# ag14774/MPILattice-Boltzmann

Measured on AMD Instinct MI355X. Metric: MLUPS, higher is better.
Workload: dtype f32; 1 GPU; synthetic 8192x8192 D2Q9-BGK deck (walls + p=0.005 random obstacles, splitmix64 seed 42), density 0.1 accel 0.005 omega 1.85; nx=8192, ny=8192, partitioning=single GPU, loop=single, macro_k=0, launches_per_exchange=1, step_allreduce=False, kernel=lbm_multi_kernel<4>

## Files before the change

### mpilattice-boltzmann_amd/csrc/kernels/multi.h

```cpp
#pragma once
#include "common.h"

namespace {

#ifndef LBM_MTY
#define LBM_MTY 16
#define LBM_MLANES 512
#endif
#ifndef LBM_MWAVES
#define LBM_MWAVES 6
#endif
#ifndef LBM_MTY4
#define LBM_MTY4 13
#endif
#ifndef LBM_MTY4T
#define LBM_MTY4T 24
#define LBM_MLANES4T 768
#endif
constexpr int kMTX = 64, kMTXNarrow = 32, kMTY = LBM_MTY, kMTY4 = LBM_MTY4, kMTY4Tall = LBM_MTY4T, kMLanes = LBM_MLANES, kMLanes4Tall = LBM_MLANES4T,
              kMaxMultiSteps = 4,
              kMaxGhost = 32,
              kMaxGroup = 8;
constexpr int kMinMultiTY = kMTY < kMTY4 ? (kMTY < kMTY4Tall ? kMTY : kMTY4Tall) : (kMTY4 < kMTY4Tall ? kMTY4 : kMTY4Tall);
constexpr int kGeomStd = 0, kGeomNarrow = 1, kGeomTall = 2;
constexpr int geom_tx(int g) { return g == kGeomNarrow ? kMTXNarrow : kMTX; }
constexpr int multi_ty(int k, int g) { return k >= 4 ? (g == kGeomTall ? kMTY4Tall : kMTY4) : kMTY; }
constexpr int multi_lanes(int k, int g) { return (k >= 4 && g == kGeomTall) ? kMLanes4Tall : kMLanes; }
constexpr int geom_for(int k, int g) { return (g == kGeomTall && k < 4) ? kGeomStd : g; }

constexpr int multi_ex(int ey) { return 2 * ((ey + 1) / 2); }
#if LBM_TILE_STAMPS
#define LBM_MSTAMP(i) do { if (blockIdx.x == (gridDim.x >> 1) && threadIdx.x == 0) g_tile_stamps[i] = __builtin_amdgcn_s_memtime(); } while (0)
#else
#define LBM_MSTAMP(i) do { } while (0)
#endif

template <int K, int GEOM = kGeomStd>
struct MultiGeom {
  static constexpr int TX = geom_tx(GEOM);
  static constexpr int TY = multi_ty(K, GEOM);
  static constexpr int LANES = multi_lanes(K, GEOM);
  static constexpr int EY = K - 1, EX = multi_ex(K - 1);
  static constexpr int W = TX + 2 * EX, H = TY + 2 * EY;
  static constexpr int cells = W * H;
  static constexpr size_t lds_bytes = sizeof(float) * 9 * cells + sizeof(double) * K * (LANES / 64) + (K >= 2 ? cells / 2 : 0);
  static constexpr int blocks_per_cu = lds_bytes * 8 <= 160 * 1024 ? 8 : static_cast<int>(160 * 1024 / lds_bytes);
  static constexpr int waves_per_simd = blocks_per_cu * (LANES / 64) / 4 < LBM_MWAVES ? (blocks_per_cu * (LANES / 64) / 4 < 1 ? 1 : blocks_per_cu * (LANES / 64) / 4) : LBM_MWAVES;
};

struct MultiArgs {
  const float* src;
  float* dst;
  const float* srck[9];
  float* dstk[9];
  const uint32_t* mask;
  size_t ps;
  int nx;
  int row_first, rows_compute;
  int rows_storage;
  int count_first, count_end;
  int y_periodic;
  int y0_global, ny_global;
  int tiles_x;
  int tile_begin, tile_count, tile_begin2, tile_count2;
  int ntiles_total;
  int xcd_remap;
  float omega, accel_w1, accel_w2;
  int accel_row;
  int accel_last;
  double* partials_out;
  const double* prev_partials;
  int n_prev, n_prev_vecs;
  double* sums;
  int* counter;
  unsigned long long* ready[2];
  unsigned long long ready_epoch;
  const unsigned long long* wait_ready;
  long long timeout_ticks;
  int* err;
  int keep_x0, keep_x1, cx0, cx1;
  unsigned long long* ready_x[2];
  int nrect;
  struct Rect { int ty0, tx0, ntx, count; } rect[4];
  int nblocks;
};

template <int W>
__device__ __forceinline__ void store_pair(float* plane, int k, int row, int fx, f2 v)
{
  if (k == 0 || k == 2 || k == 4) {
    *reinterpret_cast<f2*>(plane + row + fx) = v;
  } else {
    plane[row + (fx >> 1)] = v.y;
    plane[row + (fx >> 1) + W / 2] = v.x;
  }
}

constexpr int kPartPlain = 0, kPartGhost = 1, kPartReady = 2, kPartTile = 3;
template <int K, int TERMS, int GEOM, int PART>
__global__ void __launch_bounds__((MultiGeom<K, GEOM>::LANES), (MultiGeom<K, GEOM>::waves_per_simd)) lbm_multi_kernel(const MultiArgs a)
{
  using G = MultiGeom<K, GEOM>;
  constexpr int TX = G::TX, EX = G::EX, EY = G::EY, W = G::W, WH = G::W / 2, kCells = G::cells, kLanes = G::LANES, kWaves = kLanes / 64, TY = G::TY;
  extern __shared__ __attribute__((aligned(16))) float lds[];
  double* red = reinterpret_cast<double*>(lds + 9 * kCells);
  uint8_t* pair_flags = reinterpret_cast<uint8_t*>(red + K * kWaves);
  const int tid = threadIdx.x;

  if (blockIdx.x == 0) {
    if constexpr (PART == kPartReady) {
      if (a.ready_epoch != 0ull && tid == 0) {
        for (int d = 0; d < 2; ++d) __hip_atomic_store(a.ready[d], a.ready_epoch, __ATOMIC_RELAXED, __HIP_MEMORY_SCOPE_SYSTEM);
      }
    }
    if constexpr (PART == kPartTile) {
      if (a.ready_epoch != 0ull && tid == 0) {
        for (int d = 0; d < 2; ++d) __hip_atomic_store(a.ready[d], a.ready_epoch, __ATOMIC_RELAXED, __HIP_MEMORY_SCOPE_SYSTEM);
        for (int d = 0; d < 2; ++d) __hip_atomic_store(a.ready_x[d], a.ready_epoch, __ATOMIC_RELAXED, __HIP_MEMORY_SCOPE_SYSTEM);
      }
    }
    for (int v = 0; v < a.n_prev_vecs; ++v) {
      double s = 0.0;
      for (int i = tid; i < a.n_prev; i += kLanes) s += a.prev_partials[static_cast<size_t>(v) * a.n_prev + i];
      s = wave_sum(s);
      __syncthreads();
      if ((tid & 63) == 0) red[tid >> 6] = s;
      __syncthreads();
      if (tid == 0) {
        double t = 0.0;
        for (int w = 0; w < kWaves; ++w) t += red[w];
        a.sums[*a.counter + v] = t;
      }
    }
    __syncthreads();
    if (tid == 0 && a.n_prev_vecs > 0) *a.counter += a.n_prev_vecs;
    if constexpr (PART == kPartReady) {
      if (a.wait_ready && tid == 0) p2p_wait_flags(a.wait_ready, nullptr, 2, a.ready_epoch, 0ull, a.timeout_ticks, a.err, false);
    }
    if constexpr (PART == kPartTile) {
      if (a.wait_ready && tid == 0) p2p_wait_flags(a.wait_ready, nullptr, 4, a.ready_epoch, 0ull, a.timeout_ticks, a.err, false);
    }
    return;
  }

  LBM_MSTAMP(0);
  int b = blockIdx.x - 1;
  if (a.xcd_remap) {
    const int nb = gridDim.x - 1, per = nb >> 3;
    b = (b & 7) * per + (b >> 3);
  }
  if constexpr (PART == kPartTile) {
    if (b >= a.nblocks) return;
  }
  int tile_of_block = b < a.tile_count ? a.tile_begin + b : a.tile_begin2 + (b - a.tile_count);
  if constexpr (PART == kPartTile) {
    if (a.nrect > 0) {
      int q = b, ty0 = a.rect[0].ty0, tx0 = a.rect[0].tx0, ntx = a.rect[0].ntx;
      if (a.nrect > 1 && q >= a.rect[0].count) {
        q -= a.rect[0].count; ty0 = a.rect[1].ty0; tx0 = a.rect[1].tx0; ntx = a.rect[1].ntx;
        if (a.nrect > 2 && q >= a.rect[1].count) {
          q -= a.rect[1].count; ty0 = a.rect[2].ty0; tx0 = a.rect[2].tx0; ntx = a.rect[2].ntx;
          if (a.nrect > 3 && q >= a.rect[2].count) { q -= a.rect[2].count; ty0 = a.rect[3].ty0; tx0 = a.rect[3].tx0; ntx = a.rect[3].ntx; }
        }
      }
      const int rr = q / ntx;
      tile_of_block = (ty0 + rr) * a.tiles_x + tx0 + (q - rr * ntx);
    }
  }
  const int tile = tile_of_block;
  const int ty = tile / a.tiles_x, tx = tile - ty * a.tiles_x;
  const int x0 = tx * TX;
  const int sy0 = a.row_first + ty * TY;
  const int nx = a.nx;
  constexpr bool XR = PART == kPartTile;
  const int rows_storage = (PART == kPartGhost || PART == kPartTile) ? a.rows_storage : a.rows_compute + 2 * a.row_first;
  [[maybe_unused]] const int row_end = a.row_first + a.rows_compute;
  const int tile_row_base = sy0 * nx;
  const int grid_cells = rows_storage * nx;
  constexpr int ksteps = K;
  double acc[K];
  float acc_lo[K];
#pragma unroll
  for (int i = 0; i < K; ++i) { acc[i] = 0.0; acc_lo[i] = 0.0f; }

  bool tile_accel;
  {
    int d = (a.accel_row - (a.y0_global + ty * TY - EY)) % a.ny_global;
    if (d < 0) d += a.ny_global;
    tile_accel = d < G::H || a.ny_global < G::H;
  }
  auto on_accel_row = [&](int sr) {
    int g = a.y0_global + sr - a.row_first;
    if (g < 0) g += a.ny_global; else if (g >= a.ny_global) g -= a.ny_global;
    return g == a.accel_row;
  };

  auto k_substeps = [&](auto count_c) __attribute__((always_inline)) {
    constexpr bool COUNT = decltype(count_c)::value;
    {
      const int ey = ksteps - 1, ex = multi_ex(ey);
      const int wp = (TX + 2 * ex) / 2;
      const int np = wp * (TY + 2 * ey);
      const bool inner = x0 - EX >= 2 && x0 + TX + EX + 2 <= nx && sy0 - EY >= 1 && sy0 + TY + EY + 1 <= rows_storage &&
                         sy0 + TY <= a.row_first + a.rows_compute;
  #pragma unroll 1
      for (int i = tid; i < np; i += kLanes) {
        const int ry = i / wp, rp = i - ry * wp;
        const int fx = EX - ex + 2 * rp, fy = EY - ey + ry;
        int gx = x0 + fx - EX;
        int sr = sy0 + fy - EY;
        int cell = tile_row_base + __mul24(fy - EY, nx) + gx;
        int d_south = -nx, d_north = nx;
        if (!inner) {
          if (gx < 0) { gx += nx; cell += nx; } else if (gx >= nx) { gx -= nx; cell -= nx; }
          if (!a.y_periodic && sr + 1 >= rows_storage) {
            if (ksteps > 1) pair_flags[(fy * W + fx) >> 1] = 0;
            continue;
          }
          if (a.y_periodic) {
            if (sr < 0) { sr += rows_storage; cell += grid_cells; } else if (sr >= rows_storage) { sr -= rows_storage; cell -= grid_cells; }
            if (sr == 0) d_south = grid_cells - nx;
            if (sr + 1 >= rows_storage) d_north = nx - grid_cells;
          }
        }
        const uint32_t o_here = 4u * static_cast<uint32_t>(cell);
        const uint32_t o_south = 4u * static_cast<uint32_t>(cell + d_south);
        const uint32_t o_north = 4u * static_cast<uint32_t>(cell + d_north);
        f2 p[9];
        p[0] = at_byte<f2>(a.srck[0], o_here);
        p[2] = at_byte<f2>(a.srck[2], o_south);
        p[4] = at_byte<f2>(a.srck[4], o_north);
        p[1] = at_byte<f2u>(a.srck[1] - 1, o_here);
        p[5] = at_byte<f2u>(a.srck[5] - 1, o_south);
        p[8] = at_byte<f2u>(a.srck[8] - 1, o_north);
        p[3] = at_byte<f2u>(a.srck[3] + 1, o_here);
        p[6] = at_byte<f2u>(a.srck[6] + 1, o_south);
        p[7] = at_byte<f2u>(a.srck[7] + 1, o_north);
        if (!inner) {
          if (gx == 0) {
            p[1].x = at_byte<float>(a.srck[1] + nx - 1, o_here); p[5].x = at_byte<float>(a.srck[5] + nx - 1, o_south);
            p[8].x = at_byte<float>(a.srck[8] + nx - 1, o_north);
          }
          if (gx == nx - 2) {
            p[3].y = at_byte<float>(a.srck[3] + 2 - nx, o_here); p[6].y = at_byte<float>(a.srck[6] + 2 - nx, o_south);
            p[7].y = at_byte<float>(a.srck[7] + 2 - nx, o_north);
          }
        }
        const uint32_t mbits = (at_byte<uint32_t>(a.mask, 4u * (static_cast<uint32_t>(cell) >> 5)) >> (cell & 31)) & 3u;
        f2 out[9];
        const int srow = sy0 + fy - EY;
        const bool owned_rows = fx >= EX && fx < EX + TX && fy >= EY && fy < EY + TY &&
                                (inner || (x0 + fx - EX < nx && sy0 + fy - EY < a.row_first + a.rows_compute));
        const bool counted_rows = COUNT ? (owned_rows && srow >= a.count_first && srow < a.count_end) : owned_rows;
        bool owned = owned_rows, counted = counted_rows;
        if constexpr (XR && COUNT) {
          const int gxo = x0 + fx - EX;
          owned = owned_rows && gxo >= a.keep_x0 && gxo < a.keep_x1;
          counted = counted_rows && owned && gxo >= a.cx0 && gxo < a.cx1;
        }
        bool accel_row_here = false;
        if (tile_accel) accel_row_here = on_accel_row(sr);
        acc[0] += finish_pair_lo<TERMS>(p, mbits, a.omega, tile_accel, (ksteps > 1 || a.accel_last) && accel_row_here, a.accel_w1, a.accel_w2, counted ? mbits : 3u, out, acc_lo[0]);
        if (ksteps > 1) {
  #pragma unroll
          for (int k = 0; k < 9; ++k) store_pair<W>(lds + k * kCells, k, fy * W, fx, out[k]);
          pair_flags[(fy * W + fx) >> 1] = static_cast<uint8_t>(mbits | (owned ? 4u : 0u) | (accel_row_here ? 8u : 0u) | 16u | ((COUNT && counted) ? 32u : 0u));
        } else if (owned) {
  #pragma unroll
          for (int k = 0; k < 9; ++k) __builtin_nontemporal_store(out[k], &at_byte<f2>(a.dstk[k], o_here));
        }
      }
    }
    LBM_MSTAMP(1);
    if constexpr (K >= 2) {
      __syncthreads();
      LBM_MSTAMP(2);
      auto in_lds_substep = [&](const int j) __attribute__((always_inline)) {
        const int ey = ksteps - j, ex = multi_ex(ey);
        const int wp = (TX + 2 * ex) / 2;
        const int rows = TY + 2 * ey;
        const int rpp = kLanes / wp;
        const bool last = j == ksteps;
        const int rd = (j - 2) * W, wr = (j - 1) * W;
        const int ry = tid / wp, rp = tid - ry * wp;
        const int fx = EX - ex + 2 * rp;
        for (int r0 = 0; r0 < rows; r0 += rpp) {
          f2 outs[9];
          int slot = -1;
          const bool in_region = ry < rpp && r0 + ry < rows;
          if (__builtin_amdgcn_ballot_w64(in_region) != 0ull) {
            const int fy = EY - ey + (in_region ? r0 + ry : 0);
            const int cf = fy * W + fx;
            const uint32_t fl = pair_flags[cf >> 1];
            const bool lane_on = in_region && (fl & 16u);
            const int ci = cf - rd;
            const int cs = fy * W + (fx >> 1) - rd;
            f2 p[9];
            p[0] = *reinterpret_cast<const f2*>(lds + 0 * kCells + ci);
            p[2] = *reinterpret_cast<const f2*>(lds + 2 * kCells + ci - W);
            p[4] = *reinterpret_cast<const f2*>(lds + 4 * kCells + ci + W);
            p[1] = f2{lds[1 * kCells + cs - 1], lds[1 * kCells + cs + WH]};
            p[5] = f2{lds[5 * kCells + cs - W - 1], lds[5 * kCells + cs - W + WH]};
            p[8] = f2{lds[8 * kCells + cs + W - 1], lds[8 * kCells + cs + W + WH]};
            p[3] = f2{lds[3 * kCells + cs], lds[3 * kCells + cs + WH + 1]};
            p[6] = f2{lds[6 * kCells + cs - W], lds[6 * kCells + cs - W + WH + 1]};
            p[7] = f2{lds[7 * kCells + cs + W], lds[7 * kCells + cs + W + WH + 1]};
            const bool owned = lane_on && (fl & 4u);
            const bool counted = COUNT ? (lane_on && (fl & 32u)) : owned;
            float term_lo = 0.0f;
            const double term = finish_pair_lo<TERMS>(p, fl & 3u, a.omega, tile_accel, (!last || a.accel_last) && (fl & 8u), a.accel_w1, a.accel_w2,
                                                      counted ? (fl & 3u) : 3u, outs, term_lo);
  #pragma unroll
            for (int m = 1; m < K; ++m)
              if (m == j - 1) { acc[m] += term; acc_lo[m] += term_lo; }
            slot = !lane_on ? -1 : last ? (owned ? tile_row_base + __mul24(fy - EY, nx) + x0 + fx - EX : -1) : fy * W - wr;
          }
          if (!last) {
            __syncthreads();
            if (slot >= 0) {
  #pragma unroll
              for (int k = 0; k < 9; ++k) store_pair<W>(lds + k * kCells, k, slot, fx, outs[k]);
            }
          } else if (slot >= 0) {
  #pragma unroll
            for (int k = 0; k < 9; ++k) __builtin_nontemporal_store(outs[k], &at_byte<f2>(a.dstk[k], 4u * static_cast<uint32_t>(slot)));
          }
        }
        if (!last) __syncthreads();
        LBM_MSTAMP(1 + j);
      };
  #pragma unroll
      for (int j = 2; j <= K; ++j) in_lds_substep(j);
    }

  };
  if constexpr (PART == kPartGhost) {
    if (sy0 >= a.count_first && sy0 + TY <= a.count_end) k_substeps(std::false_type{});
    else k_substeps(std::true_type{});
  } else if constexpr (PART == kPartTile) {
    if (sy0 >= a.count_first && sy0 + TY <= a.count_end && x0 >= a.cx0 && x0 + TX <= a.cx1) k_substeps(std::false_type{});
    else k_substeps(std::true_type{});
  } else {
    k_substeps(std::false_type{});
  }

  if constexpr (TERMS == kTermsCompensated) {
#pragma unroll
    for (int i = 0; i < K; ++i) acc[i] += static_cast<double>(acc_lo[i]);
  }
  if constexpr (K == 1) {
    const double w = wave_sum(acc[0]);
    if ((tid & 63) == 0) red[tid >> 6] = w;
  } else {
    static_assert(K <= 4, "wave_sum_vec4 carries four steps");
    const double w = wave_sum_vec4(acc[0], acc[1], K > 2 ? acc[2] : 0.0, K > 3 ? acc[K > 3 ? 3 : 0] : 0.0);
    const int q = wave_sum_slot<4>(tid & 63);
    if ((tid & 15) == 0 && q < K) red[q * kWaves + (tid >> 6)] = w;
  }
  lds_barrier();
  if (tid < ksteps) {
    double t = 0.0;
    for (int w = 0; w < kWaves; ++w) t += red[tid * kWaves + w];
    a.partials_out[static_cast<size_t>(tid) * a.ntiles_total + tile] = t;
  }
  LBM_MSTAMP(2 + K);
}

}
```

Before: 239,700 MLUPS.

## Keep owned cell pairs in registers across fused substeps for K=4 tall tiles

Adds an owned-lanes path for the K=4 tall geometry. Each lane owns one interior cell pair for all substeps and keeps its rest population in a register, while a shrinking halo ring is recomputed by the remaining lanes. Flags for owned cells stay in registers, and the loop over the halo is replaced by at most one ring pair per lane. This is meant to cut LDS traffic, loop overhead and index math, at the cost of extra register pressure and a second barrier per substep.

```diff
diff --git a/mpilattice-boltzmann_amd/csrc/kernels/multi.h b/mpilattice-boltzmann_amd/csrc/kernels/multi.h
--- a/mpilattice-boltzmann_amd/csrc/kernels/multi.h
+++ b/mpilattice-boltzmann_amd/csrc/kernels/multi.h
@@ -46,6 +46,8 @@
   static constexpr size_t lds_bytes = sizeof(float) * 9 * cells + sizeof(double) * K * (LANES / 64) + (K >= 2 ? cells / 2 : 0);
   static constexpr int blocks_per_cu = lds_bytes * 8 <= 160 * 1024 ? 8 : static_cast<int>(160 * 1024 / lds_bytes);
   static constexpr int waves_per_simd = blocks_per_cu * (LANES / 64) / 4 < LBM_MWAVES ? (blocks_per_cu * (LANES / 64) / 4 < 1 ? 1 : blocks_per_cu * (LANES / 64) / 4) : LBM_MWAVES;
+  static constexpr bool owned_lanes = K == 4 && GEOM == kGeomTall;
+  static constexpr int ring_pairs(int j) { return 2 * (K - j) * (TX / 2 + multi_ex(K - j)) + TY * multi_ex(K - j); }
 };
 
 struct MultiArgs {
@@ -96,6 +98,16 @@
   }
 }
 
+__device__ __forceinline__ void accelerate_pair(f2 (&out)[9], uint32_t mbits, bool accel, float w1, float w2)
+{
+#pragma unroll
+  for (int j = 0; j < 2; ++j) {
+    const bool go = accel && !((mbits >> j) & 1u) && out[3][j] - w1 > 0.0f && out[6][j] - w2 > 0.0f && out[7][j] - w2 > 0.0f;
+    out[1][j] = go ? out[1][j] + w1 : out[1][j]; out[5][j] = go ? out[5][j] + w2 : out[5][j]; out[8][j] = go ? out[8][j] + w2 : out[8][j];
+    out[3][j] = go ? out[3][j] - w1 : out[3][j]; out[6][j] = go ? out[6][j] - w2 : out[6][j]; out[7][j] = go ? out[7][j] - w2 : out[7][j];
+  }
+}
+
 constexpr int kPartPlain = 0, kPartGhost = 1, kPartReady = 2, kPartTile = 3;
 template <int K, int TERMS, int GEOM, int PART>
 __global__ void __launch_bounds__((MultiGeom<K, GEOM>::LANES), (MultiGeom<K, GEOM>::waves_per_simd)) lbm_multi_kernel(const MultiArgs a)
@@ -195,14 +207,15 @@
     return g == a.accel_row;
   };
 
+  const bool inner = x0 - EX >= 2 && x0 + TX + EX + 2 <= nx && sy0 - EY >= 1 && sy0 + TY + EY + 1 <= rows_storage &&
+                     sy0 + TY <= a.row_first + a.rows_compute;
+
   auto k_substeps = [&](auto count_c) __attribute__((always_inline)) {
     constexpr bool COUNT = decltype(count_c)::value;
     {
       const int ey = ksteps - 1, ex = multi_ex(ey);
       const int wp = (TX + 2 * ex) / 2;
       const int np = wp * (TY + 2 * ey);
-      const bool inner = x0 - EX >= 2 && x0 + TX + EX + 2 <= nx && sy0 - EY >= 1 && sy0 + TY + EY + 1 <= rows_storage &&
-                         sy0 + TY <= a.row_first + a.rows_compute;
   #pragma unroll 1
       for (int i = tid; i < np; i += kLanes) {
         const int ry = i / wp, rp = i - ry * wp;
@@ -334,17 +347,184 @@
     }
 
   };
+
+  auto owned_substeps = [&](auto count_c) __attribute__((always_inline)) {
+    constexpr bool COUNT = decltype(count_c)::value;
+    constexpr int TP = TX / 2;
+    static_assert(TP * TY == kLanes && G::ring_pairs(1) <= kLanes, "one owned pair and at most one ring pair per lane and sub-step");
+    auto ring_pos = [&](auto jc, const int i, int& fx, int& fy) __attribute__((always_inline)) {
+      constexpr int ey = K - decltype(jc)::value, ex = multi_ex(ey), ep = ex / 2, wp = TP + ep * 2, band = ey * wp;
+      if (i < 2 * band) {
+        const bool top = i >= band;
+        const int q = top ? i - band : i, ry = q / wp, rp = q - ry * wp;
+        fy = top ? EY + TY + ry : EY - ey + ry;
+        fx = EX - ex + 2 * rp;
+      } else {
+        const int q = i - 2 * band, ry = q / (2 * ep), c = q - ry * (2 * ep);
+        fy = EY + ry;
+        fx = EX - ex + 2 * (c < ep ? c : c + TP);
+      }
+    };
+    auto relax = [&](const f2 (&p)[9], const uint32_t mbits, const bool accel, const uint32_t skip, f2 (&out)[9]) __attribute__((always_inline)) {
+      const double term = finish_pair<TERMS>(p, mbits, a.omega, false, false, a.accel_w1, a.accel_w2, skip, out);
+      if (tile_accel) accelerate_pair(out, mbits, accel, a.accel_w1, a.accel_w2);
+      return term;
+    };
+    auto pull = [&](const int fx, const int fy, f2 (&p)[9], uint32_t& mbits, int& sr) __attribute__((always_inline)) -> bool {
+      int gx = x0 + fx - EX;
+      sr = sy0 + fy - EY;
+      int cell = tile_row_base + __mul24(fy - EY, nx) + gx;
+      int d_south = -nx, d_north = nx;
+      if (!inner) {
+        if (gx < 0) { gx += nx; cell += nx; } else if (gx >= nx) { gx -= nx; cell -= nx; }
+        if (!a.y_periodic && sr + 1 >= rows_storage) return false;
+        if (a.y_periodic) {
+          if (sr < 0) { sr += rows_storage; cell += grid_cells; } else if (sr >= rows_storage) { sr -= rows_storage; cell -= grid_cells; }
+          if (sr == 0) d_south = grid_cells - nx;
+          if (sr + 1 >= rows_storage) d_north = nx - grid_cells;
+        }
+      }
+      const uint32_t o_here = 4u * static_cast<uint32_t>(cell);
+      const uint32_t o_south = 4u * static_cast<uint32_t>(cell + d_south);
+      const uint32_t o_north = 4u * static_cast<uint32_t>(cell + d_north);
+      p[0] = at_byte<f2>(a.srck[0], o_here);
+      p[2] = at_byte<f2>(a.srck[2], o_south);
+      p[4] = at_byte<f2>(a.srck[4], o_north);
+      p[1] = at_byte<f2u>(a.srck[1] - 1, o_here);
+      p[5] = at_byte<f2u>(a.srck[5] - 1, o_south);
+      p[8] = at_byte<f2u>(a.srck[8] - 1, o_north);
+      p[3] = at_byte<f2u>(a.srck[3] + 1, o_here);
+      p[6] = at_byte<f2u>(a.srck[6] + 1, o_south);
+      p[7] = at_byte<f2u>(a.srck[7] + 1, o_north);
+      if (!inner) {
+        if (gx == 0) {
+          p[1].x = at_byte<float>(a.srck[1] + nx - 1, o_here); p[5].x = at_byte<float>(a.srck[5] + nx - 1, o_south);
+          p[8].x = at_byte<float>(a.srck[8] + nx - 1, o_north);
+        }
+        if (gx == nx - 2) {
+          p[3].y = at_byte<float>(a.srck[3] + 2 - nx, o_here); p[6].y = at_byte<float>(a.srck[6] + 2 - nx, o_south);
+          p[7].y = at_byte<float>(a.srck[7] + 2 - nx, o_north);
+        }
+      }
+      mbits = (at_byte<uint32_t>(a.mask, 4u * (static_cast<uint32_t>(cell) >> 5)) >> (cell & 31)) & 3u;
+      return true;
+    };
+    const int py = tid / TP, ofx = EX + 2 * (tid - py * TP), ofy = EY + py;
+    f2 own0 = f2{0.0f, 0.0f};
+    uint32_t ofl = 0;
+  #pragma unroll 1
+    for (int item = 0; item < 2; ++item) {
+      const bool own = item == 0;
+      if (!own && tid >= G::ring_pairs(1)) break;
+      int fx = ofx, fy = ofy;
+      if (!own) ring_pos(std::integral_constant<int, 1>{}, tid, fx, fy);
+      f2 p[9];
+      uint32_t mbits = 0, fl = 0;
+      int sr = 0;
+      if (pull(fx, fy, p, mbits, sr)) {
+        const int srow = sy0 + fy - EY;
+        const bool kept_rows = own && (inner || (x0 + fx - EX < nx && srow < a.row_first + a.rows_compute));
+        const bool counted_rows = COUNT ? (kept_rows && srow >= a.count_first && srow < a.count_end) : kept_rows;
+        bool kept = kept_rows, counted = counted_rows;
+        if constexpr (XR && COUNT) {
+          const int gxo = x0 + fx - EX;
+          kept = kept_rows && gxo >= a.keep_x0 && gxo < a.keep_x1;
+          counted = counted_rows && kept && gxo >= a.cx0 && gxo < a.cx1;
+        }
+        bool accel_row_here = false;
+        if (tile_accel) accel_row_here = on_accel_row(sr);
+        f2 out[9];
+        const double term = relax(p, mbits, accel_row_here, counted ? mbits : 3u, out);
+  #pragma unroll
+        for (int k = 1; k < 9; ++k) store_pair<W>(lds + k * kCells, k, fy * W, fx, out[k]);
+        fl = mbits | (kept ? 4u : 0u) | (accel_row_here ? 8u : 0u) | 16u | ((COUNT && counted) ? 32u : 0u);
+        if (own) {
+          acc[0] = term;
+          own0 = out[0];
+        } else {
+          store_pair<W>(lds, 0, fy * W, fx, out[0]);
+        }
+      }
+      if (own) ofl = fl;
+      else pair_flags[(fy * W + fx) >> 1] = static_cast<uint8_t>(fl);
+    }
+    LBM_MSTAMP(1);
+    __syncthreads();
+    LBM_MSTAMP(2);
+    auto in_lds_substep = [&](auto jc) __attribute__((always_inline)) {
+      constexpr int j = decltype(jc)::value;
+      constexpr bool last = j == K;
+      constexpr int rd = (j - 2) * W, wr = (j - 1) * W;
+      auto read_pair = [&](const int fx, const int fy, f2 (&p)[9]) __attribute__((always_inline)) {
+        const int ci = fy * W + fx - rd, cs = fy * W + (fx >> 1) - rd;
+        p[2] = *reinterpret_cast<const f2*>(lds + 2 * kCells + ci - W);
+        p[4] = *reinterpret_cast<const f2*>(lds + 4 * kCells + ci + W);
+        p[1] = f2{lds[1 * kCells + cs - 1], lds[1 * kCells + cs + WH]};
+        p[5] = f2{lds[5 * kCells + cs - W - 1], lds[5 * kCells + cs - W + WH]};
+        p[8] = f2{lds[8 * kCells + cs + W - 1], lds[8 * kCells + cs + W + WH]};
+        p[3] = f2{lds[3 * kCells + cs], lds[3 * kCells + cs + WH + 1]};
+        p[6] = f2{lds[6 * kCells + cs - W], lds[6 * kCells + cs - W + WH + 1]};
+        p[7] = f2{lds[7 * kCells + cs + W], lds[7 * kCells + cs + W + WH + 1]};
+      };
+      f2 p[9], outs[9];
+      read_pair(ofx, ofy, p);
+      p[0] = own0;
+      const uint32_t mbits = ofl & 3u;
+      const bool counted = COUNT ? (ofl & 32u) != 0u : (ofl & 4u) != 0u;
+      acc[j - 1] = relax(p, mbits, (!last || a.accel_last) && (ofl & 8u), counted ? mbits : 3u, outs);
+      own0 = outs[0];
+      if constexpr (!last) {
+        f2 q[9];
+        int rfx = 0, rfy = 0;
+        uint32_t rfl = 0;
+        const bool ring = tid < G::ring_pairs(j);
+        if (ring) {
+          ring_pos(jc, tid, rfx, rfy);
+          rfl = pair_flags[(rfy * W + rfx) >> 1];
+          read_pair(rfx, rfy, q);
+          q[0] = *reinterpret_cast<const f2*>(lds + rfy * W + rfx - rd);
+        }
+        __syncthreads();
+        if (ofl & 16u) {
+  #pragma unroll
+          for (int k = 1; k < 9; ++k) store_pair<W>(lds + k * kCells, k, ofy * W - wr, ofx, outs[k]);
+        }
+        if (ring) {
+          f2 routs[9];
+          relax(q, rfl & 3u, (rfl & 8u) != 0u, 3u, routs);
+          if (rfl & 16u) {
+  #pragma unroll
+            for (int k = 0; k < 9; ++k) store_pair<W>(lds + k * kCells, k, rfy * W - wr, rfx, routs[k]);
+          }
+        }
+        __syncthreads();
+      } else if (ofl & 4u) {
+        const uint32_t o = 4u * static_cast<uint32_t>(tile_row_base + __mul24(py, nx) + x0 + ofx - EX);
+  #pragma unroll
+        for (int k = 0; k < 9; ++k) __builtin_nontemporal_store(outs[k], &at_byte<f2>(a.dstk[k], o));
+      }
+      LBM_MSTAMP(1 + j);
+    };
+    in_lds_substep(std::integral_constant<int, 2>{});
+    if constexpr (K >= 3) in_lds_substep(std::integral_constant<int, K >= 3 ? 3 : 2>{});
+    if constexpr (K >= 4) in_lds_substep(std::integral_constant<int, K >= 4 ? 4 : 2>{});
+  };
+  auto substeps = [&](auto count_c) __attribute__((always_inline)) {
+    if constexpr (G::owned_lanes) owned_substeps(count_c);
+    else k_substeps(count_c);
+  };
+
   if constexpr (PART == kPartGhost) {
-    if (sy0 >= a.count_first && sy0 + TY <= a.count_end) k_substeps(std::false_type{});
-    else k_substeps(std::true_type{});
+    if (sy0 >= a.count_first && sy0 + TY <= a.count_end) substeps(std::false_type{});
+    else substeps(std::true_type{});
   } else if constexpr (PART == kPartTile) {
-    if (sy0 >= a.count_first && sy0 + TY <= a.count_end && x0 >= a.cx0 && x0 + TX <= a.cx1) k_substeps(std::false_type{});
-    else k_substeps(std::true_type{});
+    if (sy0 >= a.count_first && sy0 + TY <= a.count_end && x0 >= a.cx0 && x0 + TX <= a.cx1) substeps(std::false_type{});
+    else substeps(std::true_type{});
   } else {
-    k_substeps(std::false_type{});
-  }
-
-  if constexpr (TERMS == kTermsCompensated) {
+    substeps(std::false_type{});
+  }
+
+  if constexpr (TERMS == kTermsCompensated && !G::owned_lanes) {
 #pragma unroll
     for (int i = 0; i < K; ++i) acc[i] += static_cast<double>(acc_lo[i]);
   }
```

Result: faster. 252,400 MLUPS, median of 6 (+5.3%).
